# cuMF/cumf_als

Measured on AMD Instinct MI355X. Metric: ratings/sec per ALS half-iteration (Netflix f=100); RMSE vs reference, higher is better.
Workload: dtype f32 (bf16x3-split products on the bf16 matrix pipe, fp32 accumulate); 1 GPU; netflix-shape synthetic ratings 17770x480189, nnz=99072112, f=100, lambda=0.048, solver=lu, X_BATCH=1 THETA_BATCH=1, fused Gram+solve; step=update-X + update-Theta (two half-iterations)

## Files before the change

### cumf_als_amd/csrc/als_capi.cpp

```cpp
#include <hip/hip_runtime.h>

#include <cxxabi.h>

#include <algorithm>
#include <cmath>
#include <cstdint>
#include <cstdio>
#include <cstdlib>
#include <cstring>
#include <vector>

#include "als_internal.h"
#include "cg.h"
#include "cumf_als_capi.h"

using namespace cumf;

namespace {

#if CUMF_ABLATE
int g_debug_switches = -1;
int debug_switches() {
  if (g_debug_switches < 0) g_debug_switches = getenv("CUMF_ALS_DBG") ? atoi(getenv("CUMF_ALS_DBG")) : 0;
  return g_debug_switches;
// ... 112 lines not shown
    return (int)hipErrorInvalidValue;
  }
  if (!cumf_fused_available(f, solver)) {
    fprintf(stderr, "cumf_als_update_fused: f = %d with this solver needs the materialising path "
                    "(cumf_get_hermitian + cumf_*_solve_batched): the fused LU serves even f <= %d, the fused CG "
                    "too except in gram mode exact (the full system in LDS, f <= %d)\n", f, kMaxF, kVecLd);
    return (int)hipErrorInvalidValue;
  }
  ScratchLease lease;
  KernelArgs a = base_args(p, colidx, val, gather, f, lambda);
  a.update = update;
  a.cg_iters = cg_iters;
  a.sse_bins = sse_bins;
  const int mode = (solver == CUMF_SOLVER_LU) ? kModeLU : kModeCG;
  const Route r = route_for(f, mode, plan_facts(p), switches());
  PlanLists lists{};
  int rc = plan_lists(p, &lists, static_cast<hipStream_t>(stream), r.whole == kSolveTileBuffer);
  if (!rc && r.table == kTableF16Words) rc = fast_words(p, gather, f, static_cast<hipStream_t>(stream), &a);
  if (!rc && r.table == kTablePlanes) rc = pre_words(p, gather, f, static_cast<hipStream_t>(stream), &a);
  if (rc) return rc;
  CUMF_HIP_CHECK(launch_half_iteration(a, mode, r, lists, static_cast<hipStream_t>(stream)));
  return 0;
}
}

extern "C" int cumf_als_update_fused(const cumf_plan_t* p, const int* colidx, const float* val, const float* gather,
                                     float* update, int f, float lambda, int solver, int cg_iters, void* stream) {
  return update_fused_impl(p, colidx, val, gather, update, f, lambda, solver, cg_iters, nullptr, stream);
}

extern "C" int cumf_fused_sse_available(const cumf_plan_t* p, int solver) {
  if (!p || (solver != CUMF_SOLVER_CG && solver != CUMF_SOLVER_LU)) return 0;
  return route_for(p->f, solver == CUMF_SOLVER_LU ? kModeLU : kModeCG, plan_facts(p), switches()).sse;
}

extern "C" int cumf_als_update_fused_sse(const cumf_plan_t* p, const int* colidx, const float* val, const float* gather,
                                         float* update, int f, float lambda, int solver, int cg_iters, double* sse_bins,
                                         void* stream) {
  if (!sse_bins || !cumf_fused_sse_available(p, solver)) {
    fprintf(stderr, "cumf_als_update_fused_sse: not available for this plan (cumf_fused_sse_available)\n");
    return (int)hipErrorInvalidValue;
  }
  return update_fused_impl(p, colidx, val, gather, update, f, lambda, solver, cg_iters, sse_bins, stream);
}

namespace {
int get_hermitian_any(const char* who, const cumf_plan_t* p, const int* colidx, const float* val, const float* gather,
                      void* tt, float* rhs, int f, float lambda, void* stream, int storage) {
  if (!p || f != p->f) {
    fprintf(stderr, "%s: plan/f mismatch\n", who);
    return (int)hipErrorInvalidValue;
  }
  ScratchLease lease;
  KernelArgs a = base_args(p, colidx, val, gather, f, lambda);
  a.tt = static_cast<float*>(tt);
  a.tt_half = storage == 1;
  a.tt_packed = storage == 2;
  a.rhs = rhs;
  const Route r = route_for(f, kModeMaterialize, plan_facts(p), switches());
  if (r.path == kPathGeneric) {
    if (storage != 0) {
      fprintf(stderr, "%s: f = %d is above the tile kernels' range (%d): only the fp32 f x f batch (cumf_get_hermitian)\n", who, f, kMaxF);
      return (int)hipErrorInvalidValue;
    }
    CUMF_HIP_CHECK(launch_gram_generic(a, p->n_items, static_cast<hipStream_t>(stream)));
    return 0;
// ... 232 lines not shown
```

### cumf_als_amd/csrc/als_internal.h

```cpp
#ifndef CUMF_ALS_INTERNAL_H_
#define CUMF_ALS_INTERNAL_H_

#include <hip/hip_runtime.h>

#include <algorithm>
#include <cstddef>
#include <type_traits>

#ifndef CUMF_ABLATE
#define CUMF_ABLATE 0
#endif

namespace cumf {

constexpr int kThreads = 256;
constexpr int kStage = 32;
constexpr int kVecLd = 128;
constexpr int kMaxFusedNB = 9;
constexpr int kMaxF = 207;
constexpr int kMaxFAny = 512;
constexpr int kMaxWaveNB = 7;
constexpr int kMaxFusedLuWaveNB = 9;

enum { kModeCG = 0, kModeLU = 1, kModeMaterialize = 2, kModeLUExact = 3, kModeCGHalf = 4 };
// ... 32 lines not shown
  float* update;
  float* tt;
  float* rhs;
  int tt_half;
  int tt_packed;
  int dense_slots;
  int whole_only;
  long long row_begin;
  int f;
  float lambda;
  int cg_iters;
  int dbg;
  int fast_words;
  int* fast_flag;
  int pre_words;
  unsigned pre_pitch;
  double* sse_bins;
  const float* gather_f32;
  int no_pack;
};
constexpr int kSseBins = 1024;

struct PlanLists {
  long n_items, n_mrows;
  long n_citems, n_witems;
  const int *c_row, *c_len, *c_slot, *c_rowlen;
  const long long* c_begin;
  const int *w_row, *w_len, *w_rowlen;
  const long long* w_begin;
  float* part2;
  long part2_rows;
  double chunk_share;
  long n_short;
};
constexpr int kShortRow = 32;
bool short_cg_available(int f);
hipError_t launch_short_cg(const KernelArgs& a, long n_items, hipStream_t stream);
hipError_t launch_solve_batched(const float* A, const float* b, float* x, long batch, int f, int mode, int cg_iters,
                                hipStream_t stream);
enum { kGramAuto = 0, kGramExact = 1, kGramFast = 2 };
enum { kArithSplit3 = 0, kArithFast = 1, kArithPre = 2, kArithPrePk = 3, kArithSplitPk = 4 };

struct Switches {
  int gram;
  int presplit;
  double presplit_mb;
  bool splitpk;
  bool short_cg;
  bool batched;
  bool wave_solve;
  bool lu_exact;
};
Switches switches();
void set_gram_mode(int mode);
void set_presplit_mode(int mode);

struct PlanFacts {
  int nb;
  long n_mrows, n_citems, n_witems;
  double chunk_share;
  long n_short;
  long gather_rows;
};
enum Path {
  kPathNone,
  kPathGeneric,
  kPathWorkgroup,
  kPathOneWave,
  kPathTwoWave,
};
enum Table { kTableNone, kTablePlanes, kTableF16Words };
enum Solve {
  kSolveInKernel,
  kSolveTileBuffer,
  kSolveReduce,
  kSolveWaveCG,
};
struct Route {
  Path path;
  int arith;
  int fc;
  Table table;
  bool chunk_first;
  long n_short;
  Solve chunked;
  Solve whole;
  bool sse;
};
Route route_for(int f, int mode, const PlanFacts& plan, const Switches& sw);
hipError_t launch_half_iteration(const KernelArgs& a, int mode, const Route& r, const PlanLists& lists, hipStream_t stream);

hipError_t launch_presplit(const float* src, unsigned* dst, size_t n, int* flag, hipStream_t stream);
hipError_t launch_gram_generic(const KernelArgs& a, long n_items, hipStream_t stream);
hipError_t launch_lu_global(const float* A, float* work, const float* b, float* x, long batch, int f, hipStream_t stream);
__host__ __device__ constexpr bool presplit_supported(int f) {
  return ((nb_for_f(f) == 7 || nb_for_f(f) == 5) && ((f & 15) == 0 || (f & 15) == 4)) ||
         (nb_for_f(f) > kMaxWaveNB && nb_for_f(f) <= nb_for_f(kMaxF) && (f & 3) == 0 && (f & 15) <= 8);
}
__host__ __device__ constexpr bool presplit_pays(int f) { return presplit_supported(f) && nb_for_f(f) >= 7; }
__host__ __device__ constexpr bool presplit_pays_any_size(int f) { return presplit_supported(f) && nb_for_f(f) >= 10; }
__host__ __device__ constexpr unsigned presplit_pitch(int f) {
  return 96u * (f / 16) + ((f & 15) ? (nb_for_f(f) > kMaxWaveNB ? 64u : 32u) : 0u);
}
hipError_t launch_presplit3(const float* src, void* dst, long long rows, int f, hipStream_t stream);
hipError_t launch_pack_upper(const float* full, float* packed, long batch, int f, int unpack, hipStream_t stream);
void set_last_error(int code);
void set_kernel_timing(bool on);
void note_item_kernel(const void* host_function);
const void* last_item_kernel();
hipError_t last_kernel_ms(float* item_ms, float* reduce_ms);
hipError_t kernel_ms_since_reset(float* item_ms, float* reduce_ms, int* launches);
hipError_t launch_quadratic_terms(const float* A, const float* b, const float* x, const float* reg, long batch, int f,
                                  double* out, hipStream_t stream);
hipError_t launch_sse(const float* val, const int* row, const int* col, const float* thetaT, const float* XT,
                      long count, int f, int surpass_nan, double* out, hipStream_t stream);
hipError_t launch_cg_global(const float* A, const float* b, float* x, long batch, int f, int cg_iters, bool a_half,
                            hipStream_t stream);
// ... 44 lines not shown
  kScratchRankValid = 16,
  kScratchRankMetrics = 17,
  kScratchLuWork = 18,
};
int scratch_get(hipStream_t stream, int kind, size_t bytes, void** out);
template <typename T>
CUMF_LOCAL inline int scratch(hipStream_t stream, int kind, size_t count, T** out) {
  void* q = nullptr;
  const int rc = scratch_get(stream, kind, (count ? count : 1) * sizeof(T), &q);
  *out = static_cast<T*>(q);
  return rc;
}
CUMF_LOCAL size_t scratch_capacity(hipStream_t stream, int kind);
CUMF_LOCAL int fast_flag_get(int** out);
struct ScratchLease {
  int dev = 0;
  ScratchLease();
  ~ScratchLease();
  ScratchLease(const ScratchLease&) = delete;
  ScratchLease& operator=(const ScratchLease&) = delete;
};
struct ImplicitLists;
void free_implicit_lists(ImplicitLists* lists);

}

struct cumf_plan {
  long rows = 0, row_begin = 0, row_end = 0;
  int f = 0, nb = 0, chunk = 0;
  long long plan_nnz = 0;
  long long chunk_nnz = 0;
  long n_items = 0, n_slots = 0, n_mrows = 0;
  long n_short = 0;
  int* d_item_row = nullptr;
  long long* d_item_begin = nullptr;
  int* d_item_len = nullptr;
  int* d_item_slot = nullptr;
  int* d_item_rowlen = nullptr;
  int* d_mrow_row = nullptr;
  int* d_mrow_slot0 = nullptr;
  int* d_mrow_nslots = nullptr;
  int* d_mrow_rowlen = nullptr;
  float* d_part = nullptr;
  char* d_block = nullptr;
  long n_citems = 0, n_witems = 0;
  int *d_c_row = nullptr, *d_c_len = nullptr, *d_c_slot = nullptr, *d_c_rowlen = nullptr;
  long long* d_c_begin = nullptr;
  int *d_w_row = nullptr, *d_w_len = nullptr, *d_w_rowlen = nullptr;
  long long* d_w_begin = nullptr;
  long gather_rows = 0;
  cumf::ImplicitLists* implicit = nullptr;
};

namespace cumf {

CUMF_LOCAL int plan_lists(const cumf_plan* p, PlanLists* out, hipStream_t stream, bool need_tiles);
CUMF_LOCAL PlanFacts plan_facts(const cumf_plan* p);

template <bool NOTE = false, typename... P, typename... A>
hipError_t launch_kernel(void (*kernel)(P...), dim3 grid, dim3 block, size_t lds, hipStream_t stream, const A&... args) {
  const void* fn = reinterpret_cast<const void*>(kernel);
  if (lds > 64 * 1024) {
    hipError_t e = hipFuncSetAttribute(fn, hipFuncAttributeMaxDynamicSharedMemorySize, (int)lds);
    if (e != hipSuccess) return e;
  }
  if (NOTE) note_item_kernel(fn);
// ... 23 lines not shown
```

### cumf_als_amd/csrc/als_launch.cpp

```cpp
#include <atomic>
#include <mutex>
#include <vector>

#include "als_internal.h"

namespace cumf {

namespace {
struct TimedLaunch {
  hipEvent_t ev[3];
  bool item, reduce;
};
constexpr size_t kTimedPool = 1024;
bool g_timing = false;
std::vector<TimedLaunch> g_timed;
size_t g_timed_used = 0;
TimedLaunch* g_newest = nullptr;
std::mutex g_timed_mutex;

TimedLaunch* timing_begin() {
  if (!g_timing) return nullptr;
  std::lock_guard<std::mutex> lock(g_timed_mutex);
  if (g_timed_used == kTimedPool) g_timed_used = 0;
  g_newest = &g_timed[g_timed_used++];
// ... 43 lines not shown
}

void note_item_kernel(const void* host_function) { g_last_item_kernel.store(host_function, std::memory_order_relaxed); }
const void* last_item_kernel() { return g_last_item_kernel.load(std::memory_order_relaxed); }

static hipError_t wave_items(const KernelArgs& a, int mode, const Route& r, bool whole, long n_items, hipStream_t stream) {
  return with_nb<2, kMaxNB>(nb_for_f(a.f), [&](auto nb) { return wave_item_launch<nb>(a, mode, r, whole, n_items, stream); });
}
static hipError_t reduce_rows(const KernelArgs& a, int mode, const Route& r, long n_mrows, hipStream_t stream) {
  return with_nb<1, kMaxNB>(nb_for_f(a.f), [&](auto nb) { return slice_reduce_only<nb>(a, mode, r, n_mrows, stream); });
}

static KernelArgs whole_row_items(KernelArgs a, const PlanLists& L, long w0 = 0) {
  a.item_row = L.w_row + w0, a.item_begin = L.w_begin + w0, a.item_len = L.w_len + w0;
  a.item_slot = nullptr, a.item_rowlen = L.w_rowlen + w0;
  return a;
}
static KernelArgs chunk_items(KernelArgs a, const PlanLists& L) {
  a.item_row = L.c_row, a.item_begin = L.c_begin, a.item_len = L.c_len;
  a.item_slot = L.c_slot, a.item_rowlen = L.c_rowlen;
  return a;
}

static hipError_t one_wave_items(const KernelArgs& a, int mode, const Route& r, const PlanLists& L, hipStream_t stream) {
  const KernelArgs aw = r.chunk_first ? whole_row_items(a, L) : a;
  long n_items = r.chunk_first ? L.n_witems : L.n_items;
  if (r.n_short > 0) {
    n_items -= r.n_short;
    KernelArgs as = aw;
    as.item_row += n_items, as.item_begin += n_items, as.item_len += n_items, as.item_rowlen += n_items;
    hipError_t e = launch_short_cg(as, r.n_short, stream);
    if (e != hipSuccess) return e;
  }
  if (r.chunk_first) {
    hipError_t e = wave_items(chunk_items(a, L), mode, r, false, L.n_citems, stream);
    if (e != hipSuccess) return e;
  }
  return wave_items(aw, mode, r, r.chunk_first || L.n_mrows == 0, n_items, stream);
}

static hipError_t two_wave_items(const KernelArgs& a0, int mode, const Route& r, const PlanLists& L, hipStream_t stream) {
  hipError_t e = hipSuccess;
  if (L.n_citems > 0) {
    e = wave_items(chunk_items(a0, L), kModeLU, r, false, L.n_citems, stream);
    if (e != hipSuccess) return e;
    e = reduce_rows(a0, mode, r, L.n_mrows, stream);
    if (e != hipSuccess) return e;
  }
  if (r.whole == kSolveInKernel) {
    if (L.n_witems <= 0) return hipSuccess;
    KernelArgs a = whole_row_items(a0, L);
    a.dense_slots = 0;
    return wave_items(a, mode, r, false, L.n_witems, stream);
  }
  for (long w0 = 0; w0 < L.n_witems; w0 += L.part2_rows) {
    const long cnt = L.n_witems - w0 < L.part2_rows ? L.n_witems - w0 : L.part2_rows;
    KernelArgs a = whole_row_items(a0, L, w0);
    a.dense_slots = 1;
    a.part = L.part2;
    a.mrow_row = L.w_row + w0;
    a.mrow_rowlen = L.w_rowlen + w0;
    e = wave_items(a, kModeLU, r, false, cnt, stream);
    if (e != hipSuccess) return e;
    e = reduce_rows(a, mode, r, cnt, stream);
    if (e != hipSuccess) return e;
  }
  return hipSuccess;
}

hipError_t launch_half_iteration(const KernelArgs& a, int mode, const Route& r, const PlanLists& L, hipStream_t stream) {
  const int nb = nb_for_f(a.f);
// ... 38 lines not shown
```

### cumf_als_amd/csrc/als_plan.cpp

```cpp
#include <hip/hip_runtime.h>

#include <algorithm>
#include <cstdint>
#include <cstdio>
#include <cstdlib>
#include <numeric>
#include <vector>

#include "als_internal.h"
#include "cumf_als_capi.h"

using namespace cumf;

namespace {

int default_chunk(int f, long long nnz) {
  (void)f;
  const char* e = getenv("CUMF_ALS_CHUNK");
  int c;
  if (e) {
    c = atoi(e);
  } else {
    int cus = 256;
    int dev = 0;
    if (hipGetDevice(&dev) == hipSuccess) (void)hipDeviceGetAttribute(&cus, hipDeviceAttributeMultiprocessorCount, dev);
    const long long slots = (long long)(cus > 0 ? cus : 256) * 4;
    const long long want = nnz / (slots * 12);
    c = (int)std::min<long long>(8192, std::max<long long>(2048, want));
  }
  if (c < kStage) c = kStage;
  return (c / kStage) * kStage;
}

}

extern "C" int cumf_plan_create(cumf_plan_t** out, const void* rowptr_host, int rowptr_is_64, long rows,
                                long row_begin, long row_end, int f, int chunk) {
  if (!out || !rowptr_host || rows < 0 || row_begin < 0 || row_end > rows || row_begin > row_end) {
    fprintf(stderr, "cumf_plan_create: invalid arguments\n");
    return (int)hipErrorInvalidValue;
  }
  if (f <= 0 || f > kMaxFAny || (f % 2) != 0) {
    fprintf(stderr, "cumf_plan_create: f = %d unsupported (need even f <= %d)\n", f, kMaxFAny);
    return (int)hipErrorInvalidValue;
  }
  auto rp = [&](long i) -> long long {
    return rowptr_is_64 ? static_cast<const long long*>(rowptr_host)[i]
                        : static_cast<long long>(static_cast<const int*>(rowptr_host)[i]);
  };
  if (chunk <= 0) chunk = default_chunk(f, rp(rows) - rp(0));
  if (f > kMaxF) {
    long long longest = 0;
    for (long u = row_begin; u < row_end; ++u) longest = std::max(longest, rp(u + 1) - rp(u));
    chunk = (int)std::min<long long>(0x7fffffe0LL, std::max<long long>(longest, kStage));
    chunk = ((chunk + kStage - 1) / kStage) * kStage;
  }
  chunk = std::max(kStage, (chunk / kStage) * kStage);

  std::vector<int> item_row, item_len, item_slot, item_rowlen;
  std::vector<long long> item_begin;
  std::vector<int> mrow_row, mrow_slot0, mrow_nslots, mrow_rowlen;
  {
    const size_t guess = (size_t)(row_end - row_begin) + (size_t)((rp(row_end) - rp(row_begin)) / chunk) + 16;
    item_row.reserve(guess), item_len.reserve(guess), item_slot.reserve(guess), item_rowlen.reserve(guess);
    item_begin.reserve(guess);
  }
  long n_slots = 0;
  for (long u = row_begin; u < row_end; ++u) {
    const long long s = rp(u), e = rp(u + 1);
    const long long len = e - s;
    if (len < 0 || len > 0x7fffffffLL) {
      fprintf(stderr, "cumf_plan_create: row %ld has invalid length %lld\n", u, len);
      return (int)hipErrorInvalidValue;
    }
    if (len <= chunk) {
      item_row.push_back((int)u);
      item_begin.push_back(s);
      item_len.push_back((int)len);
      item_slot.push_back(-1);
      item_rowlen.push_back((int)len);
    } else {
      const int nchunks = len == 0 ? 1 : (int)((len + chunk - 1) / chunk);
      mrow_row.push_back((int)u);
      mrow_slot0.push_back((int)n_slots);
      mrow_nslots.push_back(nchunks);
      mrow_rowlen.push_back((int)len);
      for (int c = 0; c < nchunks; ++c) {
        const long long b = s + (long long)c * chunk;
        item_row.push_back((int)u);
        item_begin.push_back(b);
        item_len.push_back((int)std::max<long long>(0, std::min<long long>(chunk, e - b)));
        item_slot.push_back((int)(n_slots + c));
        item_rowlen.push_back((int)len);
      }
      n_slots += nchunks;
    }
  }
  const size_t n_it = item_row.size();
  std::vector<long> order(n_it);
  static const int order_mode = getenv("CUMF_ALS_ORDER") ? atoi(getenv("CUMF_ALS_ORDER")) : 0;
  long n_short = 0;
  if (order_mode == 0) {
    auto bucket = [&](size_t i) -> size_t {
      const bool is_short = item_slot[i] < 0 && item_len[i] <= kShortRow;
      return is_short ? (size_t)chunk + 1 + (size_t)(kShortRow - item_len[i]) : (size_t)(chunk - item_len[i]);
    };
    std::vector<long> start((size_t)chunk + kShortRow + 3, 0);
    for (size_t i = 0; i < n_it; ++i) {
      ++start[bucket(i) + 1];
      n_short += item_slot[i] < 0 && item_len[i] <= kShortRow;
    }
    for (size_t k = 1; k < start.size(); ++k) start[k] += start[k - 1];
    for (size_t i = 0; i < n_it; ++i) order[(size_t)start[bucket(i)]++] = (long)i;
  } else {
    std::iota(order.begin(), order.end(), 0L);
  }

  cumf_plan* p = new cumf_plan();
  p->rows = rows;
  p->row_begin = row_begin;
  p->row_end = row_end;
  p->f = f;
  p->nb = nb_for_f(f);
  p->chunk = chunk;
  p->plan_nnz = rp(row_end) - rp(row_begin);
  p->n_items = (long)n_it;
  p->n_short = n_short;
  p->n_slots = n_slots;
  p->n_mrows = (long)mrow_row.size();
  for (size_t i = 0; i < n_it; ++i) {
    if (item_slot[i] >= 0) {
      ++p->n_citems;
      p->chunk_nnz += item_len[i];
    }
  }
  p->n_witems = p->n_items - p->n_citems;
  *out = nullptr;

  const size_t ni = n_it, nm = mrow_row.size(), nc = (size_t)p->n_citems, nw = (size_t)p->n_witems;
  size_t off = 0;
  auto piece = [&](size_t count, size_t elem) {
    const size_t at = off;
    off += (count * elem + 255) & ~(size_t)255;
    return at;
  };
  const size_t o_item_row = piece(ni, 4), o_item_begin = piece(ni, 8), o_item_len = piece(ni, 4), o_item_slot = piece(ni, 4),
               o_item_rowlen = piece(ni, 4), o_mrow_row = piece(nm, 4), o_mrow_slot0 = piece(nm, 4),
               o_mrow_nslots = piece(nm, 4), o_mrow_rowlen = piece(nm, 4), o_c_row = piece(nc, 4), o_c_begin = piece(nc, 8),
               o_c_len = piece(nc, 4), o_c_slot = piece(nc, 4), o_c_rowlen = piece(nc, 4), o_w_row = piece(nw, 4),
               o_w_begin = piece(nw, 8), o_w_len = piece(nw, 4), o_w_rowlen = piece(nw, 4);
  std::vector<char> host(off ? off : 256);
  auto ints = [&](size_t o) { return reinterpret_cast<int*>(host.data() + o); };
  auto longs = [&](size_t o) { return reinterpret_cast<long long*>(host.data() + o); };
  {
    size_t ic = 0, iw = 0;
    for (size_t k = 0; k < ni; ++k) {
      const size_t i = (size_t)order[k];
      ints(o_item_row)[k] = item_row[i];
      longs(o_item_begin)[k] = item_begin[i];
      ints(o_item_len)[k] = item_len[i];
// ... 37 lines not shown
  auto dlongs = [&](size_t o, size_t count) { return count ? reinterpret_cast<long long*>(p->d_block + o) : nullptr; };
  p->d_item_row = dints(o_item_row, ni), p->d_item_begin = dlongs(o_item_begin, ni), p->d_item_len = dints(o_item_len, ni);
  p->d_item_slot = dints(o_item_slot, ni), p->d_item_rowlen = dints(o_item_rowlen, ni);
  p->d_mrow_row = dints(o_mrow_row, nm), p->d_mrow_slot0 = dints(o_mrow_slot0, nm);
  p->d_mrow_nslots = dints(o_mrow_nslots, nm), p->d_mrow_rowlen = dints(o_mrow_rowlen, nm);
  p->d_c_row = dints(o_c_row, nc), p->d_c_begin = dlongs(o_c_begin, nc), p->d_c_len = dints(o_c_len, nc);
  p->d_c_slot = dints(o_c_slot, nc), p->d_c_rowlen = dints(o_c_rowlen, nc);
  p->d_w_row = dints(o_w_row, nw), p->d_w_begin = dlongs(o_w_begin, nw), p->d_w_len = dints(o_w_len, nw);
  p->d_w_rowlen = dints(o_w_rowlen, nw);
  if (n_slots > 0) {
    const size_t tiles = (size_t)p->nb * (p->nb + 1) / 2;
    PLAN_CHECK(hipMalloc(reinterpret_cast<void**>(&p->d_part), (size_t)n_slots * tiles * 256 * sizeof(float)));
  }
#undef PLAN_CHECK
  *out = p;
  return 0;
}

extern "C" int cumf_plan_destroy(cumf_plan_t* p) {
  if (!p) return 0;
  if (p->d_block) (void)hipFree(p->d_block);
  if (p->d_part) (void)hipFree(p->d_part);
  free_implicit_lists(p->implicit);
  delete p;
  return 0;
}

extern "C" int cumf_plan_set_gather_rows(cumf_plan_t* p, long gather_rows) {
  if (!p || gather_rows < 0) return (int)hipErrorInvalidValue;
  p->gather_rows = gather_rows;
  return 0;
}

extern "C" int cumf_plan_info(const cumf_plan_t* p, long info[4]) {
  if (!p || !info) return (int)hipErrorInvalidValue;
  info[0] = p->n_items;
  info[1] = p->n_slots;
  info[2] = p->n_mrows;
  info[3] = p->chunk;
  return 0;
}

int cumf::plan_lists(const cumf_plan_t* p, PlanLists* out, hipStream_t stream, bool need_tiles) {
  const size_t tile_bytes = (size_t)p->nb * (p->nb + 1) / 2 * 256 * sizeof(float);
  float* part2 = nullptr;
  long rows = 0;
  if (need_tiles && p->n_witems > 0) {
    static const double cap_gb = getenv("CUMF_ALS_TILE_BUFFER_GB") ? atof(getenv("CUMF_ALS_TILE_BUFFER_GB")) : 48.0;
    size_t cap = (size_t)(cap_gb * (double)(1ull << 30));
    size_t free_b = 0, total_b = 0;
    if (hipMemGetInfo(&free_b, &total_b) == hipSuccess) {
      const size_t mine = scratch_capacity(stream, kScratchTiles);
      cap = std::min(cap, (free_b + mine) / 2);
    }
    if (cap < ((size_t)2 << 30)) cap = (size_t)2 << 30;
    rows = (long)std::min<size_t>((size_t)p->n_witems, cap / tile_bytes);
    if (rows < 1) rows = 1;
    void* q = nullptr;
    const int rc = scratch_get(stream, kScratchTiles, (size_t)rows * tile_bytes, &q);
    if (rc) return rc;
    part2 = static_cast<float*>(q);
  }
  *out = PlanLists{p->n_items,  p->n_mrows, p->n_citems, p->n_witems, p->d_c_row,    p->d_c_len,  p->d_c_slot,
                   p->d_c_rowlen, p->d_c_begin, p->d_w_row,  p->d_w_len,  p->d_w_rowlen, p->d_w_begin, part2,
                   rows,          p->plan_nnz > 0 ? (double)p->chunk_nnz / (double)p->plan_nnz : 0.0, p->n_short};
  return 0;
}

PlanFacts cumf::plan_facts(const cumf_plan_t* p) {
  return PlanFacts{p->nb, p->n_mrows, p->n_citems, p->n_witems,
                   p->plan_nnz > 0 ? (double)p->chunk_nnz / (double)p->plan_nnz : 0.0, p->n_short, p->gather_rows};
}
```

### cumf_als_amd/csrc/als_route.cpp

```cpp
#include <cstdlib>

#include "als_internal.h"
#include "cumf_als_capi.h"

namespace cumf {

namespace {
int g_gram_mode = -1;
int g_presplit_mode = -2;
}

void set_gram_mode(int mode) { g_gram_mode = (mode == kGramExact || mode == kGramFast) ? mode : kGramAuto; }
void set_presplit_mode(int mode) { g_presplit_mode = mode; }

Switches switches() {
  if (g_gram_mode < 0) {
    const char* e = getenv("CUMF_ALS_GRAM");
    g_gram_mode = (e && (e[0] == 'e' || e[0] == 'E')) ? kGramExact : (e && (e[0] == 'f' || e[0] == 'F')) ? kGramFast : kGramAuto;
  }
  if (g_presplit_mode == -2) {
    const char* e = getenv("CUMF_ALS_PRESPLIT");
    g_presplit_mode = (e && e[0] == '0') ? CUMF_PRESPLIT_OFF : (e && e[0] == '1') ? CUMF_PRESPLIT_ON
                      : (e && e[0] == '2') ? CUMF_PRESPLIT_VERIFY : CUMF_PRESPLIT_AUTO;
  }
  static const double presplit_mb = getenv("CUMF_ALS_PRESPLIT_MB") ? atof(getenv("CUMF_ALS_PRESPLIT_MB")) : 64.0;
  static const bool splitpk = !(getenv("CUMF_ALS_SPLITPK") && *getenv("CUMF_ALS_SPLITPK") == '0');
  static const bool short_cg = !getenv("CUMF_ALS_SHORT_CG") || atoi(getenv("CUMF_ALS_SHORT_CG")) != 0;
  const char* lu_exact = getenv("CUMF_ALS_LU_EXACT");
  return Switches{g_gram_mode,
                  g_presplit_mode,
                  presplit_mb,
                  splitpk,
                  short_cg,
                  !getenv("CUMF_ALS_NO_BATCHED"),
                  !getenv("CUMF_ALS_NO_WAVE_SOLVE"),
                  lu_exact && atoi(lu_exact) != 0};
}

static bool presplit_wanted(int f, long gather_rows, const Switches& sw) {
  if (sw.presplit == CUMF_PRESPLIT_OFF || sw.gram != kGramAuto || !presplit_supported(f) || gather_rows <= 0) return false;
  if (sw.presplit == CUMF_PRESPLIT_ON || sw.presplit == CUMF_PRESPLIT_VERIFY) return true;
  return presplit_pays_any_size(f) || (presplit_pays(f) && (double)gather_rows * presplit_pitch(f) <= sw.presplit_mb * 1048576.0);
}

Route route_for(int f, int mode, const PlanFacts& p, const Switches& sw) {
  Route r{};
  const int nb = nb_for_f(f);
  const bool wave_gram = sw.gram != kGramExact;
  if (f > kMaxF)
    r.path = mode == kModeMaterialize ? kPathGeneric : kPathNone;
  else if (wave_gram && nb >= 2 && nb <= kMaxWaveNB)
    r.path = kPathOneWave;
  else if (wave_gram && sw.batched && nb > kMaxWaveNB)
    r.path = kPathTwoWave;
  else
    r.path = (mode == kModeMaterialize || fused_supported(f, mode)) ? kPathWorkgroup : kPathNone;
  const bool one = r.path == kPathOneWave, wave = one || r.path == kPathTwoWave;

  r.arith = kArithSplit3;
  if (wave && mode != kModeMaterialize) {
    if (sw.gram == kGramFast) {
      r.table = kTableF16Words;
      r.arith = kArithFast;
    } else if (presplit_wanted(f, p.gather_rows, sw)) {
      r.table = kTablePlanes;
      r.arith = (one && sw.presplit != CUMF_PRESPLIT_VERIFY) ? kArithPrePk : kArithPre;
    } else if (one && sw.splitpk && (f & 15) == 0 && sw.presplit != CUMF_PRESPLIT_OFF &&
               sw.presplit != CUMF_PRESPLIT_VERIFY) {
      r.arith = kArithSplitPk;
    }
  }
  r.fc = (one && f == 100) ? 100 : 0;

  r.chunked = (wave && mode == kModeCG && sw.wave_solve && (one || f > kVecLd)) ? kSolveWaveCG : kSolveReduce;
  r.whole = (r.path == kPathTwoWave && mode != kModeCG && !(mode == kModeLU && nb <= kMaxFusedLuWaveNB)) ? kSolveTileBuffer
                                                                                                          : kSolveInKernel;
  r.chunk_first = one && mode == kModeLU && p.n_mrows > 0 && p.n_citems > 0 && p.n_witems > 0 && p.chunk_share < 0.25;
  r.n_short = (one && mode == kModeCG && sw.short_cg && short_cg_available(f)) ? p.n_short : 0;
  r.sse = wave && mode != kModeMaterialize &&
          (p.n_mrows == 0 || r.chunked == kSolveWaveCG || (mode == kModeLU && nb >= 7));
  return r;
}

}
```

### cumf_als_amd/lib.py

```python
from __future__ import annotations

import ctypes as C
import os
import subprocess

_HERE = os.path.dirname(os.path.abspath(__file__))
CSRC = os.path.join(_HERE, "csrc")
LIB_PATH = os.environ.get("CUMF_ALS_LIB") or os.path.join(CSRC, "libALS.so")
MAIN_PATH = os.path.join(CSRC, "main")
HUGEWIKI_PATH = os.path.join(CSRC, "hugewiki")
ABLATE_LIB_PATH = os.path.join(CSRC, "libALS_ablate.so")
INCLUDE = os.path.join(os.path.dirname(_HERE), "include")

_i, _l, _f = C.c_int, C.c_long, C.c_float
_vp = _ip = _fp = C.c_void_p
_pvp = C.POINTER(C.c_void_p)
_HOST_ARGS = [_vp] * 12 + [_i, _i, _i, _l, _l, _f, _i, _i, _i, _i]
C_ABI = {
    "cumf_doALS": (_f, _HOST_ARGS),
    "cumf_doALS_ex": (_f, _HOST_ARGS + [_i] * 6 + [_vp]),
    "cumf_plan_create": (_i, [_pvp, _vp, _i, _l, _l, _l, _i, _i]),
    "cumf_plan_destroy": (_i, [_vp]),
    "cumf_plan_info": (_i, [_vp, C.POINTER(_l)]),
    "cumf_plan_set_gather_rows": (_i, [_vp, _l]),
    "cumf_gram_fast_status": (_i, [C.POINTER(_i)]),
    "cumf_fused_available": (_i, [_i, _i]),
    "cumf_als_update_fused": (_i, [_vp, _ip, _fp, _fp, _fp, _i, _f, _i, _i, _vp]),
    "cumf_fused_sse_available": (_i, [_vp, _i]),
    "cumf_als_update_fused_sse": (_i, [_vp, _ip, _fp, _fp, _fp, _i, _f, _i, _i, _vp, _vp]),
    "cumf_quadratic_sse_terms": (_i, [_fp, _fp, _fp, _fp, _l, _i, _vp, _vp]),
    "cumf_get_hermitian": (_i, [_vp, _ip, _fp, _fp, _fp, _fp, _i, _f, _vp]),
    "cumf_get_hermitian_packed": (_i, [_vp, _ip, _fp, _fp, _fp, _fp, _i, _f, _vp]),
    "cumf_get_hermitian_fp16": (_i, [_vp, _ip, _fp, _fp, _vp, _fp, _i, _f, _vp]),
    "cumf_cg_solve_batched_fp16": (_i, [_vp, _fp, _fp, _l, _i, _i, _vp]),
    "cumf_set_tt_fp16": (_i, [_i]),
    "cumf_get_tt_fp16": (_i, []),
    "cumf_cg_solve_batched": (_i, [_fp, _fp, _fp, _l, _i, _i, _vp]),
    "cumf_lu_solve_batched": (_i, [_fp, _fp, _fp, _l, _i, _vp]),
    "cumf_pack_upper": (_i, [_fp, _fp, _l, _i, _vp]),
    "cumf_unpack_upper": (_i, [_fp, _fp, _l, _i, _vp]),
    "cumf_sse": (_i, [_fp, _ip, _ip, _fp, _fp, _l, _i, _i, _vp, _vp]),
    "cumf_set_gram_mode": (_i, [_i]),
    "cumf_get_gram_mode": (_i, []),
    "cumf_set_presplit": (_i, [_i]),
    "cumf_get_presplit": (_i, []),
    "cumf_presplit_pitch": (_l, [_i]),
    "cumf_presplit_table": (_i, [_vp, _vp, _l, _i, _vp]),
    "cumf_check_gather_table": (_i, [_l, _i, _i, _i]),
    "cumf_set_kernel_timing": (_i, [_i]),
    "cumf_last_kernel_ms": (_i, [C.POINTER(_f), C.POINTER(_f)]),
    "cumf_kernel_ms_since_reset": (_i, [C.POINTER(_f), C.POINTER(_f), C.POINTER(_i)]),
    "cumf_last_kernel_name": (_i, [C.c_char_p, _i]),
    "cumf_last_error": (_i, []),
    "cumf_release_scratch": (_i, []),
    "cumf_rand_init": (None, [_fp, _l, _f, _l]),
    "cumf_widen_rowptr": (_i, [_vp, _l, _l, _vp]),
    "cumf_als_version": (_i, []),
# ... 89 lines not shown
```

### include/cumf_als_capi.h

```cpp
#ifndef CUMF_ALS_CAPI_H_
#define CUMF_ALS_CAPI_H_

#include <stdint.h>

#ifdef __cplusplus
extern "C" {
#endif

enum { CUMF_SOLVER_CG = 0, CUMF_SOLVER_LU = 1 };

float cumf_doALS(const int* csrRowIndexHostPtr, const int* csrColIndexHostPtr, const float* csrValHostPtr,
                 const int* cscRowIndexHostPtr, const int* cscColIndexHostPtr, const float* cscValHostPtr,
                 const int* cooRowIndexHostPtr, float* thetaTHost, float* XTHost,
                 const int* cooRowIndexTestHostPtr, const int* cooColIndexTestHostPtr,
                 const float* cooValHostTestPtr, const int m, const int n, const int f, const long nnz,
                 const long nnz_test, const float lambda, const int ITERS, const int X_BATCH,
                 const int THETA_BATCH, const int DEVICEID);

float cumf_doALS_ex(const int* csrRowIndexHostPtr, const int* csrColIndexHostPtr, const float* csrValHostPtr,
                    const int* cscRowIndexHostPtr, const int* cscColIndexHostPtr, const float* cscValHostPtr,
                    const int* cooRowIndexHostPtr, float* thetaTHost, float* XTHost,
                    const int* cooRowIndexTestHostPtr, const int* cooColIndexTestHostPtr,
                    const float* cooValHostTestPtr, int m, int n, int f, long nnz, long nnz_test,
                    float lambda, int ITERS, int X_BATCH, int THETA_BATCH, int DEVICEID,
                    int solver, int cg_iters, int fused, int exact_test_grid, int surpass_nan,
                    int quiet, float* rmse_log);

typedef struct cumf_plan cumf_plan_t;

int cumf_plan_create(cumf_plan_t** plan, const void* rowptr_host, int rowptr_is_64, long rows,
                     long row_begin, long row_end, int f, int chunk);
int cumf_plan_destroy(cumf_plan_t* plan);
int cumf_plan_info(const cumf_plan_t* plan, long info[4]);

int cumf_fused_available(int f, int solver);
int cumf_als_update_fused(const cumf_plan_t* plan, const int* colidx, const float* val,
                          const float* gather, float* update, int f, float lambda, int solver,
                          int cg_iters, void* stream);
#define CUMF_SSE_BINS 1024
int cumf_fused_sse_available(const cumf_plan_t* plan, int solver);
int cumf_quadratic_sse_terms(const float* A, const float* b, const float* x, const float* reg, long batch, int f,
                             double* sse_terms, void* stream);
int cumf_als_update_fused_sse(const cumf_plan_t* plan, const int* colidx, const float* val,
                              const float* gather, float* update, int f, float lambda, int solver,
                              int cg_iters, double* sse_bins, void* stream);

int cumf_get_hermitian(const cumf_plan_t* plan, const int* colidx, const float* val,
                       const float* gather, float* tt, float* rhs, int f, float lambda, void* stream);
int cumf_get_hermitian_packed(const cumf_plan_t* plan, const int* colidx, const float* val,
                              const float* gather, float* packed, float* rhs, int f, float lambda, void* stream);

int cumf_get_hermitian_fp16(const cumf_plan_t* plan, const int* colidx, const float* val, const float* gather,
                            void* tt_half, float* rhs, int f, float lambda, void* stream);
int cumf_cg_solve_batched_fp16(const void* A_half, float* x, const float* b, long batch, int f, int cg_iters,
                               void* stream);
int cumf_set_tt_fp16(int enable);
int cumf_get_tt_fp16(void);

int cumf_cg_solve_batched(const float* A, float* x, const float* b, long batch, int f, int cg_iters,
                          void* stream);

int cumf_lu_solve_batched(const float* A, const float* b, float* x, long batch, int f, void* stream);

int cumf_pack_upper(const float* full, float* packed, long batch, int f, void* stream);
int cumf_unpack_upper(const float* packed, float* full, long batch, int f, void* stream);

// ... 36 lines not shown
```

Before: 12.08 billion ratings/s.

## Solve short LU rows in dual form with a dedicated small-Gram kernel

Adds a dual-form kernel for rows with fewer ratings than features (up to 79 at f=100). It builds and solves the n×n system Θ_S Θ_Sᵀ + λI instead of the f×f normal equations, then maps back via x = Θ_Sᵀ y. The plan builder sorts these short rows and empty rows to the tail of the item order, and the launcher runs them as separate kernels. This saves Gram and LU work on the many short rows, at the cost of extra launches, an fp32 gather for the back-substitution, and a different numerical path.

```diff
diff --git a/cumf_als_amd/csrc/als_capi.cpp b/cumf_als_amd/csrc/als_capi.cpp
--- a/cumf_als_amd/csrc/als_capi.cpp
+++ b/cumf_als_amd/csrc/als_capi.cpp
@@ -168,6 +168,16 @@
 extern "C" int cumf_fused_sse_available(const cumf_plan_t* p, int solver) {
   if (!p || (solver != CUMF_SOLVER_CG && solver != CUMF_SOLVER_LU)) return 0;
   return route_for(p->f, solver == CUMF_SOLVER_LU ? kModeLU : kModeCG, plan_facts(p), switches()).sse;
+}
+
+extern "C" long cumf_plan_dual_rows(const cumf_plan_t* p, int solver) {
+  if (!p || (solver != CUMF_SOLVER_CG && solver != CUMF_SOLVER_LU)) return 0;
+  return route_for(p->f, solver == CUMF_SOLVER_LU ? kModeLU : kModeCG, plan_facts(p), switches()).n_dual;
+}
+extern "C" long cumf_route_dual_rows(int f, int solver, const long facts[5], double chunk_share) {
+  if (!facts || (solver != CUMF_SOLVER_CG && solver != CUMF_SOLVER_LU)) return 0;
+  const PlanFacts pf{nb_for_f(f), facts[0], facts[1], facts[2], chunk_share, 0, facts[3], facts[4]};
+  return route_for(f, solver == CUMF_SOLVER_LU ? kModeLU : kModeCG, pf, switches()).n_dual;
 }
 
 extern "C" int cumf_als_update_fused_sse(const cumf_plan_t* p, const int* colidx, const float* val, const float* gather,
diff --git a/cumf_als_amd/csrc/als_dual.h b/cumf_als_amd/csrc/als_dual.h
--- /dev/null
+++ b/cumf_als_amd/csrc/als_dual.h
@@ -0,0 +1,19 @@
+#pragma once
+
+namespace cumf {
+
+struct DualGeo {
+  static constexpr int NB = 5;
+  static constexpr int kRows = 16 * NB;
+  static constexpr int kPitch = 208;
+  static constexpr int kLanes = kPitch / 16;
+  static constexpr int kGroup = 4 * kPitch;
+  static constexpr int kImage = kRows * kPitch;
+  static constexpr int kStrip = kImage;
+  static constexpr int kRv = kStrip + 32 * kRows;
+  static constexpr int kY = kRv + 4 * kRows;
+  static constexpr int kBytes = kY + 4 * kRows;
+  static_assert(4 * kLanes <= 64, "four ratings fit the wave");
+};
+
+}
diff --git a/cumf_als_amd/csrc/als_dual.hip b/cumf_als_amd/csrc/als_dual.hip
--- /dev/null
+++ b/cumf_als_amd/csrc/als_dual.hip
@@ -0,0 +1,190 @@
+#include <hip/hip_runtime.h>
+
+#include "als_device.h"
+#include "als_lu_wg.h"
+#include "als_lu_blocked.h"
+#include "als_internal.h"
+#include "als_wave_gram.h"
+#include "als_wave_pre.h"
+#include "als_wave_solve.h"
+#include "als_dual.h"
+
+namespace cumf {
+
+typedef __attribute__((address_space(3))) u32x4* lds_u32x4_ptr;
+typedef __attribute__((address_space(3))) u32x2* lds_u32x2_ptr;
+
+template <int FB>
+__global__ __launch_bounds__(64, 2) void als_dual_kernel(const KernelArgs a) {
+  extern __shared__ __attribute__((aligned(16))) float smem[];
+  using G = DualGeo;
+  constexpr int NB = G::NB, NT = NB * (NB + 1) / 2, NS = FB / 2, NE = G::kRows / 4;
+  static_assert(FB % 2 == 0, "whole slices of 32 features");
+  const int lane = threadIdx.x, c = lane & 15, g = lane >> 4;
+  const int item = blockIdx.x;
+  const int row = a.item_row[item];
+  const long long begin = a.item_begin[item];
+  const int n = a.item_len[item];
+  const int rowlen = a.item_rowlen[item];
+  const int f = a.f;
+  const bool sp = (f & 15) != 0;
+  [[maybe_unused]] const unsigned pitch = a.pre_pitch;
+  char* image = reinterpret_cast<char*>(smem);
+  lds_byte_ptr lds = (lds_byte_ptr)smem;
+  float* rv = reinterpret_cast<float*>(image + G::kRv);
+  float* y = reinterpret_cast<float*>(image + G::kY);
+  const int* ib = a.colidx + begin;
+  const int top = n - 1;
+
+  int q = lane / G::kLanes;
+  const int piece = lane % G::kLanes;
+  [[maybe_unused]] const bool dma_active = q < 4 && piece < G::kLanes - 1;
+  q = q < 4 ? q : 3;
+  [[maybe_unused]] const char* lane_base = reinterpret_cast<const char*>(a.gather) + 32 * FB * (piece >> 2) + 16 * (piece & 3);
+  [[maybe_unused]] const char* zero_base = reinterpret_cast<const char*>(g_wave_zeros) + 16 * piece;
+  int idx[NE];
+#pragma unroll
+  for (int E = 0; E < NE; ++E) {
+    const int pos = 4 * E + q;
+    idx[E] = ib[pos < top ? pos : top];
+  }
+  for (int o = G::kGroup * ((n + 3) >> 2) + 16 * lane; o < G::kImage; o += 1024)
+    *reinterpret_cast<f32x4*>(image + o) = f32x4{0.f, 0.f, 0.f, 0.f};
+  for (int rho = lane; rho < G::kRows; rho += 64) {
+    const float v = a.val != nullptr ? a.val[begin + (rho < top ? rho : top)] : 0.f;
+    rv[rho] = rho < n ? v : 0.f;
+    y[rho] = 0.f;
+  }
+  auto dma_slice = [&](auto sc) {
+#if defined(__HIP_DEVICE_COMPILE__)
+    constexpr int s = decltype(sc)::value;
+    using gptr = const __attribute__((address_space(1))) void*;
+    using lptr = __attribute__((address_space(3))) void*;
+    if (dma_active) {
+      static_for<NE>([&](auto ec) {
+        constexpr int E = decltype(ec)::value;
+        if (4 * E < n) {
+          const char* src = lane_base + (unsigned long long)(unsigned)idx[E] * pitch + 64 * s;
+          src = (4 * E + q < n) ? src : zero_base;
+          __builtin_amdgcn_global_load_lds((gptr)src, (lptr)(lds + G::kGroup * E), 16, 0, 0);
+        }
+      });
+    }
+#endif
+  };
+#if defined(__HIP_DEVICE_COMPILE__)
+  if (sp) {
+    using gptr = const __attribute__((address_space(1))) void*;
+    using lptr = __attribute__((address_space(3))) void*;
+    static_for<(G::kRows + 31) / 32>([&](auto kc) {
+      constexpr int k = decltype(kc)::value;
+      const int rho = 32 * k + (lane >> 1);
+      if (rho < G::kRows) {
+        const int j = ib[rho < top ? rho : top];
+        const char* src = reinterpret_cast<const char*>(a.gather) + (unsigned long long)(unsigned)j * pitch + 96 * FB + 16 * (lane & 1);
+        src = rho < n ? src : reinterpret_cast<const char*>(g_wave_zeros) + 16 * (lane & 1);
+        __builtin_amdgcn_global_load_lds((gptr)src, (lptr)(lds + G::kStrip + 1024 * k), 16, 0, 0);
+      }
+    });
+  }
+#endif
+  dma_slice(std::integral_constant<int, 0>{});
+
+  f32x4 acc[NT];
+#pragma unroll
+  for (int t = 0; t < NT; ++t) acc[t] = f32x4{0.f, 0.f, 0.f, 0.f};
+  const lds_byte_ptr op = lds + G::kPitch * c + 16 * g;
+  static_for<NS>([&](auto sc) {
+    constexpr int s = decltype(sc)::value;
+    Planes<NB> P;
+    __builtin_amdgcn_s_waitcnt(0x0F70);
+    static_for<NB>([&](auto ic) {
+      constexpr int I = decltype(ic)::value;
+      P.h[I] = *(lds_u32x4_ptr)(op + 16 * G::kPitch * I);
+      P.m[I] = *(lds_u32x4_ptr)(op + 16 * G::kPitch * I + 64);
+      P.l[I] = *(lds_u32x4_ptr)(op + 16 * G::kPitch * I + 128);
+    });
+    __builtin_amdgcn_s_waitcnt(0xC07F);
+    if constexpr (s + 1 < NS) dma_slice(std::integral_constant<int, s + 1>{});
+    u32x4 h2[2] = {{0u, 0u, 0u, 0u}, {0u, 0u, 0u, 0u}};
+    static_for<GramSched<NB>::N>([&](auto nc) { gram_mfma_sched<NB, GramSched, decltype(nc)::value>(P, acc, h2); });
+  });
+  if (sp) {
+    const int a0 = g < 2 ? 0 : (g == 2 ? 8 : 16), a1 = g == 0 ? 0 : (g == 3 ? 16 : 8);
+    const int b0 = g == 1 ? 16 : (g == 2 ? 8 : 0), b1 = g == 1 ? 0 : (g == 2 ? 16 : 8);
+    const lds_byte_ptr st = lds + G::kStrip + 32 * c;
+    u32x4 SA[NB], SB[NB];
+    static_for<NB>([&](auto ic) {
+      constexpr int I = decltype(ic)::value;
+      const u32x2 p0 = *(lds_u32x2_ptr)(st + 512 * I + a0), p1 = *(lds_u32x2_ptr)(st + 512 * I + a1);
+      const u32x2 q0 = *(lds_u32x2_ptr)(st + 512 * I + b0), q1 = *(lds_u32x2_ptr)(st + 512 * I + b1);
+      SA[I] = u32x4{p0[0], p0[1], p1[0], p1[1]};
+      SB[I] = u32x4{q0[0], q0[1], q1[0], q1[1]};
+    });
+    static_for<NT>([&](auto tc) {
+      constexpr int t = decltype(tc)::value, I = tile_I<NB>(t), J = tile_J<NB>(t);
+      acc[t] = mfma_bf16(SA[I], SB[J], acc[t]);
+    });
+  }
+  __builtin_amdgcn_s_waitcnt(0xC07F);
+  wave_symmetrise_diag<NB>(acc, smem, lane);
+
+  const int fr = n > 16 * (NB - 1) ? n : 16 * (NB - 1);
+  const int cr = fr - 16 * (NB - 1);
+  static_for<NB>([&](auto ic) {
+    constexpr int I = decltype(ic)::value;
+    constexpr int t = tile_of<NB>(I, NB - 1);
+    const f32x4 v = *reinterpret_cast<const f32x4*>(rv + 16 * I + 4 * g);
+#pragma unroll
+    for (int r = 0; r < 4; ++r) acc[t][r] = c == cr ? v[r] : acc[t][r];
+  });
+  {
+    const float v = rv[16 * (NB - 1) + c];
+#pragma unroll
+    for (int r = 0; r < 4; ++r) acc[NT - 1][r] = 4 * g + r == cr ? v : acc[NT - 1][r];
+  }
+
+  const float reg = (float)rowlen * a.lambda;
+  const float ssq = lu_wave_blocked<NB, 0>(acc, smem, fr, reg, y, lane);
+  __syncthreads();
+
+  const bool two = lane + 64 < f;
+  float x0 = 0.f, x1 = 0.f;
+  auto fetch = [&](int pos, float& t0, float& t1, float& yv) {
+    const int rho = pos < top ? pos : top;
+    const float* trow = a.gather_f32 + (size_t)(unsigned)ib[rho] * f;
+    t0 = trow[lane];
+    t1 = two ? trow[lane + 64] : 0.f;
+    yv = pos < n ? y[rho] : 0.f;
+  };
+  for (int r0 = 0; r0 < n; r0 += 4) {
+    float ta0, ta1, ya, tb0, tb1, yb, tc0, tc1, yc, td0, td1, yd;
+    fetch(r0, ta0, ta1, ya);
+    fetch(r0 + 1, tb0, tb1, yb);
+    fetch(r0 + 2, tc0, tc1, yc);
+    fetch(r0 + 3, td0, td1, yd);
+    x0 = fmaf(ta0, ya, x0), x1 = fmaf(ta1, ya, x1);
+    x0 = fmaf(tb0, yb, x0), x1 = fmaf(tb1, yb, x1);
+    x0 = fmaf(tc0, yc, x0), x1 = fmaf(tc1, yc, x1);
+    x0 = fmaf(td0, yd, x0), x1 = fmaf(td1, yd, x1);
+  }
+  float* xg = a.update + (size_t)row * f;
+  xg[lane] = x0;
+  if (two) xg[lane + 64] = x1;
+
+  if (a.sse_bins != nullptr) {
+    const float yy = wave_sum_uniform(ssq);
+    wave_sse_add(a.sse_bins, (double)reg * (double)reg * (double)yy, rowlen, lane);
+  }
+}
+
+hipError_t launch_dual_lu(const KernelArgs& a, long n_items, hipStream_t stream) {
+  if (n_items <= 0) return hipSuccess;
+  if (dual_max_len(a.f) <= 0 || !presplit_supported(a.f) || a.pre_pitch != presplit_pitch(a.f) || a.gather_f32 == nullptr)
+    return hipErrorInvalidValue;
+  static_assert((size_t)DualGeo::kRv >= wave_lu_lds_floats<DualGeo::NB>(16 * DualGeo::NB - 1) * sizeof(float),
+                "the right-hand side and y lie behind what the elimination aliases");
+  return launch_kernel(als_dual_kernel<6>, dim3((unsigned)n_items), dim3(64), DualGeo::kBytes, stream, a);
+}
+
+}
diff --git a/cumf_als_amd/csrc/als_internal.h b/cumf_als_amd/csrc/als_internal.h
--- a/cumf_als_amd/csrc/als_internal.h
+++ b/cumf_als_amd/csrc/als_internal.h
@@ -88,10 +88,13 @@
   long part2_rows;
   double chunk_share;
   long n_short;
+  long n_dual, n_empty;
 };
 constexpr int kShortRow = 32;
 bool short_cg_available(int f);
 hipError_t launch_short_cg(const KernelArgs& a, long n_items, hipStream_t stream);
+__host__ __device__ constexpr int dual_max_len(int f) { return f / 16 + 1 == 7 ? 16 * (7 - 2) - 1 : 0; }
+hipError_t launch_dual_lu(const KernelArgs& a, long n_items, hipStream_t stream);
 hipError_t launch_solve_batched(const float* A, const float* b, float* x, long batch, int f, int mode, int cg_iters,
                                 hipStream_t stream);
 enum { kGramAuto = 0, kGramExact = 1, kGramFast = 2 };
@@ -106,6 +109,7 @@
   bool batched;
   bool wave_solve;
   bool lu_exact;
+  bool dual;
 };
 Switches switches();
 void set_gram_mode(int mode);
@@ -117,6 +121,7 @@
   double chunk_share;
   long n_short;
   long gather_rows;
+  long n_dual;
 };
 enum Path {
   kPathNone,
@@ -139,6 +144,7 @@
   Table table;
   bool chunk_first;
   long n_short;
+  long n_dual;
   Solve chunked;
   Solve whole;
   bool sse;
@@ -249,6 +255,7 @@
   long long chunk_nnz = 0;
   long n_items = 0, n_slots = 0, n_mrows = 0;
   long n_short = 0;
+  long n_dual = 0, n_empty = 0;
   int* d_item_row = nullptr;
   long long* d_item_begin = nullptr;
   int* d_item_len = nullptr;
diff --git a/cumf_als_amd/csrc/als_launch.cpp b/cumf_als_amd/csrc/als_launch.cpp
--- a/cumf_als_amd/csrc/als_launch.cpp
+++ b/cumf_als_amd/csrc/als_launch.cpp
@@ -99,11 +99,29 @@
     hipError_t e = launch_short_cg(as, r.n_short, stream);
     if (e != hipSuccess) return e;
   }
+  const long n_dual = (mode == kModeLU && a.lambda > 0.f) ? r.n_dual : 0;
+  const long n_empty = n_dual > 0 ? L.n_empty : 0;
+  auto from = [&](long i0) {
+    KernelArgs b = aw;
+    b.item_row += i0, b.item_begin += i0, b.item_len += i0, b.item_rowlen += i0;
+    if (b.item_slot) b.item_slot += i0;
+    return b;
+  };
+  if (n_dual > 0) {
+    n_items -= n_dual + n_empty;
+    hipError_t e = launch_dual_lu(from(n_items), n_dual, stream);
+    if (e != hipSuccess) return e;
+  }
   if (r.chunk_first) {
     hipError_t e = wave_items(chunk_items(a, L), mode, r, false, L.n_citems, stream);
     if (e != hipSuccess) return e;
   }
-  return wave_items(aw, mode, r, r.chunk_first || L.n_mrows == 0, n_items, stream);
+  const bool whole = r.chunk_first || L.n_mrows == 0;
+  if (n_empty > 0) {
+    hipError_t e = wave_items(from(n_items + n_dual), mode, r, whole, n_empty, stream);
+    if (e != hipSuccess) return e;
+  }
+  return wave_items(aw, mode, r, whole, n_items, stream);
 }
 
 static hipError_t two_wave_items(const KernelArgs& a0, int mode, const Route& r, const PlanLists& L, hipStream_t stream) {
diff --git a/cumf_als_amd/csrc/als_plan.cpp b/cumf_als_amd/csrc/als_plan.cpp
--- a/cumf_als_amd/csrc/als_plan.cpp
+++ b/cumf_als_amd/csrc/als_plan.cpp
@@ -32,11 +32,19 @@
   return (c / kStage) * kStage;
 }
 
-}
-
-extern "C" int cumf_plan_create(cumf_plan_t** out, const void* rowptr_host, int rowptr_is_64, long rows,
-                                long row_begin, long row_end, int f, int chunk) {
-  if (!out || !rowptr_host || rows < 0 || row_begin < 0 || row_end > rows || row_begin > row_end) {
+struct HostItems {
+  int chunk = 0;
+  std::vector<int> item_row, item_len, item_slot, item_rowlen;
+  std::vector<long long> item_begin;
+  std::vector<int> mrow_row, mrow_slot0, mrow_nslots, mrow_rowlen;
+  std::vector<long> order;
+  long n_slots = 0, n_short = 0;
+  long n_dual = 0, n_empty = 0;
+};
+
+int build_items(HostItems& h, const void* rowptr_host, int rowptr_is_64, long rows, long row_begin, long row_end, int f,
+                int chunk) {
+  if (!rowptr_host || rows < 0 || row_begin < 0 || row_end > rows || row_begin > row_end) {
     fprintf(stderr, "cumf_plan_create: invalid arguments\n");
     return (int)hipErrorInvalidValue;
   }
@@ -44,6 +52,10 @@
     fprintf(stderr, "cumf_plan_create: f = %d unsupported (need even f <= %d)\n", f, kMaxFAny);
     return (int)hipErrorInvalidValue;
   }
+  auto& item_row = h.item_row; auto& item_len = h.item_len; auto& item_slot = h.item_slot; auto& item_rowlen = h.item_rowlen;
+  auto& item_begin = h.item_begin;
+  auto& mrow_row = h.mrow_row; auto& mrow_slot0 = h.mrow_slot0; auto& mrow_nslots = h.mrow_nslots; auto& mrow_rowlen = h.mrow_rowlen;
+  auto& order = h.order;
   auto rp = [&](long i) -> long long {
     return rowptr_is_64 ? static_cast<const long long*>(rowptr_host)[i]
                         : static_cast<long long>(static_cast<const int*>(rowptr_host)[i]);
@@ -57,9 +69,6 @@
   }
   chunk = std::max(kStage, (chunk / kStage) * kStage);
 
-  std::vector<int> item_row, item_len, item_slot, item_rowlen;
-  std::vector<long long> item_begin;
-  std::vector<int> mrow_row, mrow_slot0, mrow_nslots, mrow_rowlen;
   {
     const size_t guess = (size_t)(row_end - row_begin) + (size_t)((rp(row_end) - rp(row_begin)) / chunk) + 16;
     item_row.reserve(guess), item_len.reserve(guess), item_slot.reserve(guess), item_rowlen.reserve(guess);
@@ -97,13 +106,15 @@
     }
   }
   const size_t n_it = item_row.size();
-  std::vector<long> order(n_it);
+  order.assign(n_it, 0L);
   static const int order_mode = getenv("CUMF_ALS_ORDER") ? atoi(getenv("CUMF_ALS_ORDER")) : 0;
+  const int dual_len = dual_max_len(f);
   long n_short = 0;
   if (order_mode == 0) {
     auto bucket = [&](size_t i) -> size_t {
       const bool is_short = item_slot[i] < 0 && item_len[i] <= kShortRow;
-      return is_short ? (size_t)chunk + 1 + (size_t)(kShortRow - item_len[i]) : (size_t)(chunk - item_len[i]);
+      const int len = (item_slot[i] >= 0 && item_len[i] <= dual_len && dual_len < chunk) ? dual_len + 1 : item_len[i];
+      return is_short ? (size_t)chunk + 1 + (size_t)(kShortRow - item_len[i]) : (size_t)(chunk - len);
     };
     std::vector<long> start((size_t)chunk + kShortRow + 3, 0);
     for (size_t i = 0; i < n_it; ++i) {
@@ -115,6 +126,43 @@
   } else {
     std::iota(order.begin(), order.end(), 0L);
   }
+
+  if (order_mode == 0 && dual_len > 0 && dual_len < chunk) {
+    size_t k = n_it;
+    auto whole = [&](size_t pos, int lo, int hi) {
+      const size_t i = (size_t)order[pos];
+      return item_slot[i] < 0 && item_len[i] >= lo && item_len[i] <= hi;
+    };
+    for (; k > 0 && whole(k - 1, 0, 0); --k) ++h.n_empty;
+    for (; k > 0 && whole(k - 1, 1, dual_len); --k) ++h.n_dual;
+  }
+  h.chunk = chunk;
+  h.n_slots = n_slots;
+  h.n_short = n_short;
+  return 0;
+}
+
+}
+
+extern "C" int cumf_plan_create(cumf_plan_t** out, const void* rowptr_host, int rowptr_is_64, long rows,
+                                long row_begin, long row_end, int f, int chunk) {
+  if (!out) {
+    fprintf(stderr, "cumf_plan_create: invalid arguments\n");
+    return (int)hipErrorInvalidValue;
+  }
+  HostItems h;
+  if (const int rc = build_items(h, rowptr_host, rowptr_is_64, rows, row_begin, row_end, f, chunk)) return rc;
+  chunk = h.chunk;
+  const auto& item_row = h.item_row; const auto& item_len = h.item_len; const auto& item_slot = h.item_slot;
+  const auto& item_rowlen = h.item_rowlen; const auto& item_begin = h.item_begin;
+  const auto& mrow_row = h.mrow_row; const auto& mrow_slot0 = h.mrow_slot0; const auto& mrow_nslots = h.mrow_nslots;
+  const auto& mrow_rowlen = h.mrow_rowlen; const auto& order = h.order;
+  const size_t n_it = item_row.size();
+  const long n_slots = h.n_slots, n_short = h.n_short;
+  auto rp = [&](long i) -> long long {
+    return rowptr_is_64 ? static_cast<const long long*>(rowptr_host)[i]
+                        : static_cast<long long>(static_cast<const int*>(rowptr_host)[i]);
+  };
 
   cumf_plan* p = new cumf_plan();
   p->rows = rows;
@@ -126,6 +174,7 @@
   p->plan_nnz = rp(row_end) - rp(row_begin);
   p->n_items = (long)n_it;
   p->n_short = n_short;
+  p->n_dual = h.n_dual, p->n_empty = h.n_empty;
   p->n_slots = n_slots;
   p->n_mrows = (long)mrow_row.size();
   for (size_t i = 0; i < n_it; ++i) {
@@ -229,6 +278,20 @@
   return 0;
 }
 
+extern "C" int cumf_plan_dual_facts(const void* rowptr_host, int rowptr_is_64, long rows, long row_begin, long row_end, int f,
+                                    int chunk, long facts[4], int* order_len, int* order_slot, long order_cap) {
+  if (!facts) return (int)hipErrorInvalidValue;
+  HostItems h;
+  if (const int rc = build_items(h, rowptr_host, rowptr_is_64, rows, row_begin, row_end, f, chunk)) return rc;
+  const long n = (long)h.order.size();
+  facts[0] = n, facts[1] = h.n_dual, facts[2] = n - h.n_empty - h.n_dual, facts[3] = h.n_empty;
+  for (long k = 0; k < n && k < order_cap; ++k) {
+    if (order_len) order_len[k] = h.item_len[(size_t)h.order[(size_t)k]];
+    if (order_slot) order_slot[k] = h.item_slot[(size_t)h.order[(size_t)k]];
+  }
+  return 0;
+}
+
 extern "C" int cumf_plan_info(const cumf_plan_t* p, long info[4]) {
   if (!p || !info) return (int)hipErrorInvalidValue;
   info[0] = p->n_items;
@@ -260,11 +323,13 @@
   }
   *out = PlanLists{p->n_items,  p->n_mrows, p->n_citems, p->n_witems, p->d_c_row,    p->d_c_len,  p->d_c_slot,
                    p->d_c_rowlen, p->d_c_begin, p->d_w_row,  p->d_w_len,  p->d_w_rowlen, p->d_w_begin, part2,
-                   rows,          p->plan_nnz > 0 ? (double)p->chunk_nnz / (double)p->plan_nnz : 0.0, p->n_short};
+                   rows,          p->plan_nnz > 0 ? (double)p->chunk_nnz / (double)p->plan_nnz : 0.0, p->n_short,
+                   p->n_dual,     p->n_empty};
   return 0;
 }
 
 PlanFacts cumf::plan_facts(const cumf_plan_t* p) {
   return PlanFacts{p->nb, p->n_mrows, p->n_citems, p->n_witems,
-                   p->plan_nnz > 0 ? (double)p->chunk_nnz / (double)p->plan_nnz : 0.0, p->n_short, p->gather_rows};
-}
+                   p->plan_nnz > 0 ? (double)p->chunk_nnz / (double)p->plan_nnz : 0.0, p->n_short, p->gather_rows,
+                   p->n_dual};
+}
diff --git a/cumf_als_amd/csrc/als_route.cpp b/cumf_als_amd/csrc/als_route.cpp
--- a/cumf_als_amd/csrc/als_route.cpp
+++ b/cumf_als_amd/csrc/als_route.cpp
@@ -27,6 +27,7 @@
   static const bool splitpk = !(getenv("CUMF_ALS_SPLITPK") && *getenv("CUMF_ALS_SPLITPK") == '0');
   static const bool short_cg = !getenv("CUMF_ALS_SHORT_CG") || atoi(getenv("CUMF_ALS_SHORT_CG")) != 0;
   const char* lu_exact = getenv("CUMF_ALS_LU_EXACT");
+  const char* dual = getenv("CUMF_ALS_DUAL");
   return Switches{g_gram_mode,
                   g_presplit_mode,
                   presplit_mb,
@@ -34,7 +35,8 @@
                   short_cg,
                   !getenv("CUMF_ALS_NO_BATCHED"),
                   !getenv("CUMF_ALS_NO_WAVE_SOLVE"),
-                  lu_exact && atoi(lu_exact) != 0};
+                  lu_exact && atoi(lu_exact) != 0,
+                  !dual || atoi(dual) != 0};
 }
 
 static bool presplit_wanted(int f, long gather_rows, const Switches& sw) {
@@ -77,6 +79,10 @@
                                                                                                           : kSolveInKernel;
   r.chunk_first = one && mode == kModeLU && p.n_mrows > 0 && p.n_citems > 0 && p.n_witems > 0 && p.chunk_share < 0.25;
   r.n_short = (one && mode == kModeCG && sw.short_cg && short_cg_available(f)) ? p.n_short : 0;
+  r.n_dual = (one && mode == kModeLU && r.table == kTablePlanes && r.arith == kArithPrePk && sw.gram == kGramAuto && sw.dual &&
+              dual_max_len(f) > 0)
+                 ? p.n_dual
+                 : 0;
   r.sse = wave && mode != kModeMaterialize &&
           (p.n_mrows == 0 || r.chunked == kSolveWaveCG || (mode == kModeLU && nb >= 7));
   return r;
diff --git a/cumf_als_amd/lib.py b/cumf_als_amd/lib.py
--- a/cumf_als_amd/lib.py
+++ b/cumf_als_amd/lib.py
@@ -23,6 +23,9 @@
     "cumf_plan_destroy": (_i, [_vp]),
     "cumf_plan_info": (_i, [_vp, C.POINTER(_l)]),
     "cumf_plan_set_gather_rows": (_i, [_vp, _l]),
+    "cumf_plan_dual_rows": (_l, [_vp, _i]),
+    "cumf_plan_dual_facts": (_i, [_vp, _i, _l, _l, _l, _i, _i, C.POINTER(_l), _ip, _ip, _l]),
+    "cumf_route_dual_rows": (_l, [_i, _i, C.POINTER(_l), C.c_double]),
     "cumf_gram_fast_status": (_i, [C.POINTER(_i)]),
     "cumf_fused_available": (_i, [_i, _i]),
     "cumf_als_update_fused": (_i, [_vp, _ip, _fp, _fp, _fp, _i, _f, _i, _i, _vp]),
diff --git a/include/cumf_als_capi.h b/include/cumf_als_capi.h
--- a/include/cumf_als_capi.h
+++ b/include/cumf_als_capi.h
@@ -32,6 +32,10 @@
                      long row_begin, long row_end, int f, int chunk);
 int cumf_plan_destroy(cumf_plan_t* plan);
 int cumf_plan_info(const cumf_plan_t* plan, long info[4]);
+long cumf_plan_dual_rows(const cumf_plan_t* plan, int solver);
+int cumf_plan_dual_facts(const void* rowptr_host, int rowptr_is_64, long rows, long row_begin, long row_end, int f,
+                         int chunk, long facts[4], int* order_len, int* order_slot, long order_cap);
+long cumf_route_dual_rows(int f, int solver, const long facts[5], double chunk_share);
 
 int cumf_fused_available(int f, int solver);
 int cumf_als_update_fused(const cumf_plan_t* plan, const int* colidx, const float* val,
```

Result: slower. 11.44 billion ratings/s (-5.4%).
